# rare-resilience-ai/Osteosarcoma_DiffusionModel

Hardware: AMD Instinct MI355X
Metric: synthetic patients/sec (full T-step reverse sample) (higher is better)
Workload: dtype f32; 1 GPU; reverse sampling of conditional patients, T=1000, D=2000 (50 mut + 1900 expr + 50 pathway), hidden [256,512,256], 3 scenario conditions (BASELINE config 3); patients_per_gpu=100000, T=1000, parallelism=patients sharded over 1 GPU(s), no collective, sampler=chain, chunk_rows=65536, streams=2, graph=True

## Files before the change

### osteosarcoma_diffusionmodel_amd/csrc/gemm_bf3.h

```cpp
#pragma once
#include "gemm_glds.h"
#include "epilogues.h"

namespace osd {

typedef __bf16 bf16x8 __attribute__((ext_vector_type(8)));
typedef __bf16 bf16x2 __attribute__((ext_vector_type(2)));
typedef unsigned v4u32 __attribute__((ext_vector_type(4)));
typedef __attribute__((address_space(1))) v4u32 gv4u32;

constexpr int B3_ROWS = 128;
constexpr int B3_KB = 16;
constexpr int B3_STAGE_U4 = 768;
constexpr int B3_STAGE_BYTES = B3_STAGE_U4 * 16;
constexpr int B3_SLOT_BYTES = 2 * B3_STAGE_BYTES;
#ifndef B3_RING
#define B3_RING 3
#endif
constexpr int B3_SLOTS = B3_RING;
constexpr int B3_LDS_RING_BYTES = B3_SLOTS * B3_SLOT_BYTES;
constexpr int B3_LDS_BYTES = B3_LDS_RING_BYTES + 384 * 4;

inline int64_t b3_tiles(int64_t rows) { return (rows + B3_ROWS - 1) / B3_ROWS; }
inline int b3_nkb(int K) { return (K + B3_KB - 1) / B3_KB; }
inline int64_t b3_units(int64_t rows, int K) { return b3_tiles(rows) * b3_nkb(K) * B3_STAGE_U4; }

struct Bf3Args {
  const uint4* A; int nkb;
  const uint4* B0; int nkb0;
  const uint4* B1; int nkb1;
  int F, P;
  unsigned long long* stamps;
};

__device__ __forceinline__ unsigned pk_bf16(float a, float b) {
  const bf16x2 p = {(__bf16)a, (__bf16)b};
  return __builtin_bit_cast(unsigned, p);
}
__device__ __forceinline__ float bf_lo(unsigned u) { return __uint_as_float(u << 16); }
__device__ __forceinline__ float bf_hi(unsigned u) { return __uint_as_float(u & 0xffff0000u); }

struct Split4 { uint2 p[3]; };
__device__ __forceinline__ Split4 split4(float4 v) {
  Split4 s;
  const unsigned a0 = pk_bf16(v.x, v.y), a1 = pk_bf16(v.z, v.w);
  const float rx = v.x - bf_lo(a0), ry = v.y - bf_hi(a0), rz = v.z - bf_lo(a1), rw = v.w - bf_hi(a1);
  const unsigned b0 = pk_bf16(rx, ry), b1 = pk_bf16(rz, rw);
  const float sx = rx - bf_lo(b0), sy = ry - bf_hi(b0), sz = rz - bf_lo(b1), sw = rw - bf_hi(b1);
  s.p[0] = make_uint2(a0, a1);
  s.p[1] = make_uint2(b0, b1);
  s.p[2] = make_uint2(pk_bf16(sx, sy), pk_bf16(sz, sw));
  return s;
}

__device__ __forceinline__ void stg_u4(uint4* p, uint4 v) { const v4u32 w = {v.x, v.y, v.z, v.w}; *(gv4u32*)p = w; }

__device__ __forceinline__ void b3_put_pair(uint4* __restrict__ o, int kb, int rb, float4 X, float4 Y) {
  const Split4 sx = split4(X), sy = split4(Y);
#pragma unroll
  for (int pl = 0; pl < 3; ++pl) {
    const auto r0 = __builtin_amdgcn_permlane32_swap(sx.p[pl].x, sy.p[pl].x, false, false);
    const auto r1 = __builtin_amdgcn_permlane32_swap(sx.p[pl].y, sy.p[pl].y, false, false);
    stg_u4(o + ((kb * 3 + pl) * 4 + rb) * 64, make_uint4(r0[0], r1[0], r0[1], r1[1]));
  }
}

struct B3Ctx {
  int f0;
  int fl;
  int pt, rb0;
  int p0w;
  int lane, wave;
  int F, P;
  const float* prm;
  float* xreg;
};
constexpr int B3_PRM_FLOATS = 384;

struct B3Out { uint4* planes; int nkb; };

struct B3NoState {};
struct EpiB3Base {
  typedef B3NoState State;
  static constexpr bool LOOP_RNG = false;
  static constexpr bool X_TILE = false;
};

struct EpiB3Bias : EpiB3Base {
  struct Args { const float* bias; float* out; int ldo; };
  static __device__ __forceinline__ const float* prm_ptr(const Args& a, int k) { return k == 0 ? a.bias : nullptr; }
  static __device__ __forceinline__ void apply(f32x16 (&acc)[2][2], const Args& a, const B3Ctx& c, State&) {
    const int l31 = c.lane & 31, h = c.lane >> 5;
#pragma unroll
    for (int fb = 0; fb < 2; ++fb)
#pragma unroll
      for (int q = 0; q < 4; ++q) {
        const int fo = c.fl + 32 * fb + 8 * q + 4 * h;
        const int f = c.f0 + fo;
        const float4 bv = a.bias ? *reinterpret_cast<const float4*>(c.prm + fo) : make_float4(0.f, 0.f, 0.f, 0.f);
        const float b4[4] = {bv.x, bv.y, bv.z, bv.w};
#pragma unroll
        for (int pb = 0; pb < 2; ++pb) {
          const int p = c.p0w + 32 * pb + l31;
          if (p < c.P) {
            float* row = a.out + (size_t)p * a.ldo;
#pragma unroll
            for (int r = 0; r < 4; ++r)
              if (f + r < c.F) row[f + r] = acc[fb][pb][4 * q + r] + b4[r];
          }
        }
      }
  }
};

struct EpiB3Input : EpiB3Base {
  struct Args {
    const float* bias; const float* temb; int ldt; const int* t_index; const int* t_dev; int t_imm;
    const float* cproj; int ldc; B3Out o;
  };
  static __device__ __forceinline__ const float* prm_ptr(const Args& a, int k) {
    if (k == 0) return a.bias;
    if (k == 1 && !a.t_index) return a.temb + (size_t)(a.t_dev ? *a.t_dev : a.t_imm) * a.ldt;
    return nullptr;
  }
  static __device__ __forceinline__ void apply(f32x16 (&acc)[2][2], const Args& a, const B3Ctx& c, State&) {
    const int l31 = c.lane & 31, h = c.lane >> 5;
    uint4* const ob = a.o.planes + (size_t)c.pt * a.o.nkb * B3_STAGE_U4 + c.lane;
#pragma unroll
    for (int pb = 0; pb < 2; ++pb) {
      const int p = c.p0w + 32 * pb + l31;
      const int pc = p < c.P ? p : c.P - 1;
      const float* trow = a.t_index ? a.temb + (size_t)a.t_index[pc] * a.ldt + c.f0 : nullptr;
      const float* crow = a.cproj + (size_t)pc * a.ldc + c.f0;
#pragma unroll
      for (int fb = 0; fb < 2; ++fb)
#pragma unroll
        for (int j = 0; j < 2; ++j) {
          float4 v[2];
#pragma unroll
          for (int e = 0; e < 2; ++e) {
            const int q = 2 * j + e;
            const int fo = c.fl + 32 * fb + 8 * q + 4 * h;
            const float4 bv = *reinterpret_cast<const float4*>(c.prm + fo);
            const float4 tv = trow ? ldg4(trow + fo) : *reinterpret_cast<const float4*>(c.prm + 128 + fo);
            const float4 cv = ldg4(crow + fo);
            v[e].x = ((acc[fb][pb][4 * q] + bv.x) + tv.x) + cv.x;
            v[e].y = ((acc[fb][pb][4 * q + 1] + bv.y) + tv.y) + cv.y;
            v[e].z = ((acc[fb][pb][4 * q + 2] + bv.z) + tv.z) + cv.z;
            v[e].w = ((acc[fb][pb][4 * q + 3] + bv.w) + tv.w) + cv.w;
          }
          b3_put_pair(ob, (c.f0 + c.fl + 32 * fb) / 16 + j, c.rb0 + pb, v[0], v[1]);
        }
    }
  }
};

template <int GW>
struct EpiB3Gn : EpiB3Base {
  struct Args { const float* bias; const float* gamma; const float* beta; B3Out o; };
  static __device__ __forceinline__ const float* prm_ptr(const Args& a, int k) { return k == 0 ? a.bias : (k == 1 ? a.gamma : a.beta); }
  static __device__ __forceinline__ void apply(f32x16 (&acc)[2][2], const Args& a, const B3Ctx& c, B3NoState&) {
    static_assert(GW == 32 || GW == 64, "group widths of the 256 / 512 wide trunk");
    constexpr int RPG = GW / 2;
    constexpr int NG = 32 / RPG;
    const int h = c.lane >> 5;
    uint4* const ob = a.o.planes + (size_t)c.pt * a.o.nkb * B3_STAGE_U4 + c.lane;
#pragma unroll
    for (int fb = 0; fb < 2; ++fb)
#pragma unroll
      for (int q = 0; q < 4; ++q) {
        const float4 bv = *reinterpret_cast<const float4*>(c.prm + c.fl + 32 * fb + 8 * q + 4 * h);
#pragma unroll
        for (int pb = 0; pb < 2; ++pb) {
          acc[fb][pb][4 * q] += bv.x; acc[fb][pb][4 * q + 1] += bv.y;
          acc[fb][pb][4 * q + 2] += bv.z; acc[fb][pb][4 * q + 3] += bv.w;
        }
      }
    float mean[2][NG], rstd[2][NG];
#pragma unroll
    for (int pb = 0; pb < 2; ++pb)
#pragma unroll
      for (int g = 0; g < NG; ++g) {
        float s = 0.f;
#pragma unroll
        for (int j = 0; j < RPG; ++j) { const int Li = g * RPG + j; s += acc[Li / 16][pb][Li % 16]; }
        s += swap_halves(s);
        const float m = s * (1.0f / GW);
        float qs = 0.f;
#pragma unroll
        for (int j = 0; j < RPG; ++j) { const int Li = g * RPG + j; const float d = acc[Li / 16][pb][Li % 16] - m; qs = fmaf(d, d, qs); }
        qs += swap_halves(qs);
        mean[pb][g] = m;
        rstd[pb][g] = 1.0f / sqrtf(qs * (1.0f / GW) + GN_EPS);
      }
#pragma unroll
    for (int fb = 0; fb < 2; ++fb)
#pragma unroll
      for (int j = 0; j < 2; ++j) {
        float4 gv[2], bev[2];
#pragma unroll
        for (int e = 0; e < 2; ++e) {
          const int fo = c.fl + 32 * fb + 8 * (2 * j + e) + 4 * h;
          gv[e] = *reinterpret_cast<const float4*>(c.prm + 128 + fo);
          bev[e] = *reinterpret_cast<const float4*>(c.prm + 256 + fo);
        }
#pragma unroll
        for (int pb = 0; pb < 2; ++pb) {
          float4 y[2];
#pragma unroll
          for (int e = 0; e < 2; ++e) {
            const int q = 2 * j + e;
            const int g = (fb * 16 + 4 * q) / RPG;
            const float m = mean[pb][g], r = rstd[pb][g];
            y[e].x = silu_f(fmaf((acc[fb][pb][4 * q] - m) * r, gv[e].x, bev[e].x));
            y[e].y = silu_f(fmaf((acc[fb][pb][4 * q + 1] - m) * r, gv[e].y, bev[e].y));
            y[e].z = silu_f(fmaf((acc[fb][pb][4 * q + 2] - m) * r, gv[e].z, bev[e].z));
            y[e].w = silu_f(fmaf((acc[fb][pb][4 * q + 3] - m) * r, gv[e].w, bev[e].w));
          }
          b3_put_pair(ob, (c.f0 + c.fl + 32 * fb) / 16 + j, c.rb0 + pb, y[0], y[1]);
        }
      }
  }
};

struct EpiB3Post : EpiB3Base {
  static constexpr bool LOOP_RNG = true;
  static constexpr bool X_TILE = true;
  struct Args {
    const float* bias; float* x; int ldx; const float* coef; const int* t_dev; int t_imm;
    const float* z; int ldzz; long long z_step_stride; int t_first;
    uint64_t seed; uint32_t row_offset; float* mut_mask; int mutation_dim; B3Out o;
    int x_tile;
  };
  struct State { float4 z[16]; int t; };
  static __device__ __forceinline__ const float* prm_ptr(const Args& a, int k) { return k == 0 ? a.bias : nullptr; }
  static __device__ __forceinline__ void init(State& st, const Args& a) { st.t = a.t_dev ? *a.t_dev : a.t_imm; }
  static __device__ __forceinline__ float4 draw(const Args& a, const B3Ctx& c, int t, int i) {
    const int fb = i >> 3, pb = (i >> 2) & 1, q = i & 3;
    const int p = c.p0w + 32 * pb + (c.lane & 31);
    const int f = c.f0 + c.fl + 32 * fb + 8 * q + 4 * (c.lane >> 5);
    return randn4(a.seed, a.row_offset + (uint32_t)p, (uint32_t)(f >> 2), (uint32_t)t, TAG_POSTERIOR);
  }
  static __device__ __forceinline__ bool rng_on(const Args& a, const State& st) { return st.t > 0 && !a.z && a.coef[4 * st.t + 2] != 0.f; }
  static __device__ __forceinline__ void kstep(State& st, const Args& a, const B3Ctx& c, int i) { st.z[i] = draw(a, c, st.t, i); }
  static __device__ __forceinline__ void xtile_issue(const Args& a, const B3Ctx& c) {
    const int rows = c.P - c.p0w;
    const int cmax = (c.F - (c.f0 + c.fl)) / 4 - 1;
    const unsigned dst = __builtin_amdgcn_readfirstlane(lds_addr(c.xreg));
#pragma unroll
    for (int i = 0; i < 16; ++i) {
      const int r = 4 * i + (c.lane >> 4);
      int ch = (c.lane & 15) ^ (r & 15);
      ch = ch < cmax ? ch : (cmax > 0 ? cmax : 0);
      long long row = (long long)c.p0w + (r < rows ? r : rows - 1);
      row = row > 0 ? row : 0;
      int f = c.f0 + c.fl + 4 * ch;
      f = f < c.F - 4 ? f : c.F - 4;
      glds16(a.x + row * a.ldx + f, __builtin_amdgcn_readfirstlane(dst + (unsigned)i * 1024u));
    }
  }
  static __device__ __forceinline__ void apply(f32x16 (&acc)[2][2], const Args& a, const B3Ctx& c, State& st) {
    const int l31 = c.lane & 31, h = c.lane >> 5;
    const int t = st.t;
    const float* cf = a.coef + 4 * t;
    const float cA = cf[0], cB = cf[1], cC = cf[2];
    const float* zbase = a.z ? a.z + (long long)(a.t_first - t) * a.z_step_stride : nullptr;
    const bool do_mask = t == 0 && a.mut_mask != nullptr;
    const bool zal = zbase && (a.ldzz & 3) == 0 && (reinterpret_cast<uintptr_t>(zbase) & 15) == 0;
    const int f0w = c.f0 + c.fl;
    uint4* const ob = a.o.planes + (size_t)c.pt * a.o.nkb * B3_STAGE_U4 + c.lane;
#pragma unroll
    for (int fb = 0; fb < 2; ++fb)
#pragma unroll
      for (int q = 0; q < 4; ++q) {
        const int fo = c.fl + 32 * fb + 8 * q + 4 * h;
        const int f = c.f0 + fo;
        const float4 b4 = *reinterpret_cast<const float4*>(c.prm + fo);
        const float bv[4] = {b4.x, b4.y, b4.z, b4.w};
#pragma unroll
        for (int pb = 0; pb < 2; ++pb) {
          float zv[4] = {0.f, 0.f, 0.f, 0.f};
          if (t > 0 && cC != 0.f) {
            if (zbase) {
              const int p = c.p0w + 32 * pb + l31;
              const size_t zo = (size_t)(p < c.P ? p : c.P - 1) * a.ldzz;
              if (zal && f + 3 < c.F) { const float4 z4 = ldg4(zbase + zo + f); zv[0] = z4.x; zv[1] = z4.y; zv[2] = z4.z; zv[3] = z4.w; }
              else {
#pragma unroll
                for (int r = 0; r < 4; ++r) zv[r] = f + r < c.F ? zbase[zo + f + r] : 0.f;
              }
            } else {
              const float4 z4 = st.z[(fb * 2 + pb) * 4 + q];
              zv[0] = z4.x; zv[1] = z4.y; zv[2] = z4.z; zv[3] = z4.w;
            }
          }
#pragma unroll
          for (int r = 0; r < 4; ++r) acc[fb][pb][4 * q + r] = fmaf(cB, acc[fb][pb][4 * q + r] + bv[r], cC * zv[r]);
        }
      }
    if (a.x_tile) asm volatile("s_waitcnt vmcnt(0)" ::: "memory");
#pragma unroll
    for (int fb = 0; fb < 2; ++fb) {
      if (f0w + 32 * fb >= c.F) break;
#pragma unroll
      for (int pb = 0; pb < 2; ++pb) {
        const int rl = 32 * pb + l31;
        const int p = c.p0w + rl;
        const bool prow = p < c.P;
        const int pc = prow ? p : c.P - 1;
        float* xrow = a.x + (size_t)pc * a.ldx;
#pragma unroll
        for (int j = 0; j < 2; ++j) {
          if (f0w + 32 * fb + 16 * j >= c.F) break;
          float4 o[2];
#pragma unroll
          for (int e = 0; e < 2; ++e) {
            const int q = 2 * j + e;
            const int fo = c.fl + 32 * fb + 8 * q + 4 * h;
            const int f = c.f0 + fo;
            float xv[4];
            float* xs = nullptr;
            if (a.x_tile) {
              xs = c.xreg + rl * 64 + 4 * ((8 * fb + 2 * q + h) ^ (rl & 15));
              const float4 x4 = *reinterpret_cast<const float4*>(xs);
              xv[0] = x4.x; xv[1] = x4.y; xv[2] = x4.z; xv[3] = x4.w;
            } else {
#pragma unroll
              for (int r = 0; r < 4; ++r) xv[r] = f + r < c.F ? xrow[f + r] : 0.f;
            }
            float ov[4];
#pragma unroll
            for (int r = 0; r < 4; ++r) {
              ov[r] = fmaf(cA, xv[r], acc[fb][pb][4 * q + r]);
              if (f + r >= c.F) ov[r] = 0.f;
            }
            if (do_mask && prow && f < a.mutation_dim) {
              float* mrow = a.mut_mask + (size_t)p * a.mutation_dim;
#pragma unroll
              for (int r = 0; r < 4; ++r)
                if (f + r < a.mutation_dim) mrow[f + r] = (ov[r] > 0.5f) ? 1.0f : 0.0f;
            }
            o[e] = make_float4(ov[0], ov[1], ov[2], ov[3]);
            if (a.x_tile) *reinterpret_cast<float4*>(xs) = o[e];
            else if (prow) {
#pragma unroll
              for (int r = 0; r < 4; ++r)
                if (f + r < c.F) xrow[f + r] = ov[r];
            }
          }
          b3_put_pair(ob, (f0w + 32 * fb) / 16 + j, c.rb0 + pb, o[0], o[1]);
        }
      }
    }
    if (a.x_tile) {
      const int rows = c.P - c.p0w;
      const int nch = (c.F - f0w) / 4;
#pragma unroll
      for (int i0 = 0; i0 < 16; i0 += 4) {
        float4 v[4];
#pragma unroll
        for (int k = 0; k < 4; ++k) v[k] = *reinterpret_cast<const float4*>(c.xreg + (i0 + k) * 256 + c.lane * 4);
#pragma unroll
        for (int k = 0; k < 4; ++k) {
          const int r = 4 * (i0 + k) + (c.lane >> 4);
          const int ch = (c.lane & 15) ^ (r & 15);
          if (r < rows && ch < nch) stg4(a.x + (size_t)(c.p0w + r) * a.ldx + f0w + 4 * ch, v[k]);
        }
      }
    }
  }
};

struct B3Frags { uint4 a[2][3], b[2][3]; };
#ifndef B3_LD
#define B3_LD 0
#endif
#ifndef B3_SGB_VALU
#define B3_SGB_VALU 5
#endif
#ifndef B3_EXP
#define B3_EXP 0
#endif

template <int N>
__device__ __forceinline__ void glds16s_run(gfloat_ptr sbase, unsigned voff, unsigned lds_dst) {
  static_assert(N == 3 || N == 4, "runs of 3 or 4 pieces (instruction offsets up to 3072)");
  unsigned keep;
  if constexpr (N == 3)
    asm volatile(
        "s_mov_b32 %0, m0\n\ts_mov_b32 m0, %3\n\ts_nop 4\n\t"
        "global_load_lds_dwordx4 %1, %2\n\tglobal_load_lds_dwordx4 %1, %2 offset:1024\n\tglobal_load_lds_dwordx4 %1, %2 offset:2048\n\t"
        "s_mov_b32 m0, %0"
        : "=&s"(keep) : "v"(voff), "s"(sbase), "s"(lds_dst) : "memory");
  else
    asm volatile(
        "s_mov_b32 %0, m0\n\ts_mov_b32 m0, %3\n\ts_nop 4\n\t"
        "global_load_lds_dwordx4 %1, %2\n\tglobal_load_lds_dwordx4 %1, %2 offset:1024\n\tglobal_load_lds_dwordx4 %1, %2 offset:2048\n\t"
        "global_load_lds_dwordx4 %1, %2 offset:3072\n\t"
        "s_mov_b32 m0, %0"
        : "=&s"(keep) : "v"(voff), "s"(sbase), "s"(lds_dst) : "memory");
}
__device__ __forceinline__ void glds4(const float* gsrc, unsigned lds_dst) {
  unsigned keep;
  asm volatile(
      "s_mov_b32 %0, m0\n\ts_mov_b32 m0, %2\n\ts_nop 0\n\tglobal_load_lds_dword %1, off\n\ts_mov_b32 m0, %0"
      : "=&s"(keep) : "v"(gsrc), "s"(lds_dst) : "memory");
}
template <int N> __device__ __forceinline__ void b3_wait_vm() {
  static_assert(N == 0 || N == 6 || N == 12 || N == 24, "");
  if constexpr (N == 0) asm volatile("s_waitcnt vmcnt(0)" ::: "memory");
  else if constexpr (N == 6) asm volatile("s_waitcnt vmcnt(6)" ::: "memory");
  else if constexpr (N == 12) asm volatile("s_waitcnt vmcnt(12)" ::: "memory");
  else asm volatile("s_waitcnt vmcnt(24)" ::: "memory");
}

template <class Epi, int LD, int NKB = 0>
__global__ __launch_bounds__(NTHREADS + 64 * LD, (LD || B3_RING == 2) ? 3 : 2) void gemm_bf3_kernel(Bf3Args g, typename Epi::Args ea) {
  static_assert(LD == 0 || LD == 2, "no loader waves, or one per operand");
  static_assert(NKB == 0 || NKB == 16 || NKB == 32, "unrolled lengths: 256 / 512 deep reductions");
  extern __shared__ __attribute__((aligned(16))) uint4 b3smem[];
  const int nft = (g.F + B3_ROWS - 1) / B3_ROWS;
  const int npt = (g.P + B3_ROWS - 1) / B3_ROWS;
  const int b = blockIdx.x;
  const int idx = b >> 3;
  const int ft = idx % nft;
  const int pt = (idx / nft) * 8 + (b & 7);
  if (pt >= npt) return;
  const int pt_src = (B3_EXP & 2) ? 0 : pt;

  const int tid = threadIdx.x;
  const int lane = tid & 63;
  const int wave = __builtin_amdgcn_readfirstlane(tid >> 6);
  const bool loader = LD > 0 && wave >= 4;
  const int rbA = ((wave >> 1) & 1) * 2;
  const int rbB = (wave & 1) * 2;

  const int nkb = NKB ? NKB : g.nkb;
  const gfloat_ptr Ag = uniform_ptr(reinterpret_cast<const float*>(g.A + (size_t)ft * nkb * B3_STAGE_U4));
  const gfloat_ptr B0g = uniform_ptr(reinterpret_cast<const float*>(g.B0 + (size_t)pt_src * g.nkb0 * B3_STAGE_U4));
  const gfloat_ptr B1g = uniform_ptr(reinterpret_cast<const float*>(g.B1 ? g.B1 + (size_t)pt_src * g.nkb1 * B3_STAGE_U4 : g.B0));
  const int nkb0 = g.nkb0;
  const unsigned voff = (unsigned)lane * 16u;
  const unsigned lds0 = __builtin_amdgcn_readfirstlane(lds_addr(reinterpret_cast<const float*>(b3smem)));
  float* const prm = reinterpret_cast<float*>(b3smem) + B3_LDS_RING_BYTES / 4;
  unsigned long long st_c = 0, st_r = 0;
  if (g.stamps) { st_c = __builtin_amdgcn_s_memtime(); st_r = __builtin_amdgcn_s_memrealtime(); }

  if (wave < 3) {
    const float* src = Epi::prm_ptr(ea, wave);
    if (src) {
      const int f0 = ft * B3_ROWS;
#pragma unroll
      for (int i = 0; i < 2; ++i) {
        int f = f0 + 64 * i + lane;
        f = f < g.F ? f : g.F - 1;
        glds4(src + f, __builtin_amdgcn_readfirstlane(lds_addr(prm) + (unsigned)wave * 512u + (unsigned)i * 256u));
      }
    }
  }

  auto issue_stage = [&](int st, int sl) {
    const gfloat_ptr as = Ag + (size_t)st * (B3_STAGE_BYTES / 4);
    const gfloat_ptr bs = st < nkb0 ? B0g + (size_t)st * (B3_STAGE_BYTES / 4) : B1g + (size_t)(st - nkb0) * (B3_STAGE_BYTES / 4);
    const unsigned dst = lds0 + (unsigned)sl * (unsigned)B3_SLOT_BYTES;
    if constexpr (LD == 0) {
      glds16s_run<3>(as + wave * 768, voff, __builtin_amdgcn_readfirstlane(dst + (unsigned)wave * 3072u));
      glds16s_run<3>(bs + wave * 768, voff, __builtin_amdgcn_readfirstlane(dst + (unsigned)B3_STAGE_BYTES + (unsigned)wave * 3072u));
    } else {
      const gfloat_ptr src = wave == 4 ? as : bs;
      const unsigned d = __builtin_amdgcn_readfirstlane(dst + (wave == 4 ? 0u : (unsigned)B3_STAGE_BYTES));
#pragma unroll
      for (int i = 0; i < 3; ++i) glds16s_run<4>(src + i * 1024, voff, __builtin_amdgcn_readfirstlane(d + (unsigned)i * 4096u));
    }
  };
  constexpr int PPS = LD ? 12 : 6;
  auto read_frags = [&](B3Frags& f, int sl) {
    const uint4* s = b3smem + sl * (B3_SLOT_BYTES / 16) + lane;
#pragma unroll
    for (int pl = 0; pl < 3; ++pl)
#pragma unroll
      for (int i = 0; i < 2; ++i) {
        f.a[i][pl] = s[(pl * 4 + rbA + i) * 64];
        f.b[i][pl] = s[B3_STAGE_U4 + (pl * 4 + rbB + i) * 64];
      }
  };

  int s0 = 0, s1 = 1, s2 = 2;
  if (loader) {
    issue_stage(0, 0);
    if (nkb > 1) issue_stage(1, 1);
    if (nkb > 2) issue_stage(2, 2);
    if (nkb > 2) b3_wait_vm<2 * PPS>(); else if (nkb > 1) b3_wait_vm<PPS>(); else b3_wait_vm<0>();
    asm volatile("s_barrier" ::: "memory");
    if (nkb > 2) b3_wait_vm<PPS>(); else b3_wait_vm<0>();
    asm volatile("s_barrier" ::: "memory");
    for (int s = 0; s < nkb; ++s) {
      const bool more = s + 3 < nkb && !(B3_EXP & 1);
      if (more) { issue_stage(s + 3, s0); b3_wait_vm<PPS>(); } else b3_wait_vm<0>();
      if (!(B3_EXP & 8)) asm volatile("s_barrier" ::: "memory");
      const int k = s0; s0 = s1; s1 = s2; s2 = k;
    }
    return;
  }

  f32x16 acc[2][2];
#pragma unroll
  for (int i = 0; i < 2; ++i)
#pragma unroll
    for (int j = 0; j < 2; ++j)
#pragma unroll
      for (int r = 0; r < 16; ++r) acc[i][j][r] = 0.f;

  B3Ctx ctx;
  ctx.f0 = ft * B3_ROWS; ctx.fl = rbA * 32; ctx.pt = pt; ctx.rb0 = rbB; ctx.p0w = pt * B3_ROWS + rbB * 32;
  ctx.lane = lane; ctx.wave = wave; ctx.F = g.F; ctx.P = g.P; ctx.prm = prm;
  ctx.xreg = reinterpret_cast<float*>(b3smem) + wave * 4096;
  typename Epi::State est;
  bool rng = false;
  if constexpr (Epi::LOOP_RNG) { Epi::init(est, ea); rng = NKB > 0 && Epi::rng_on(ea, est); }
  bool xt = false;
  if constexpr (Epi::X_TILE) xt = ea.x_tile != 0 && B3_RING == 3;

  auto mfma_block = [&](const B3Frags& f, bool draw, int rs) {
    constexpr int PA[6] = {2, 1, 0, 1, 0, 0};
    constexpr int PB[6] = {0, 1, 2, 0, 1, 0};
#pragma unroll
    for (int t = 0; t < 6; ++t)
#pragma unroll
      for (int i = 0; i < 2; ++i)
#pragma unroll
        for (int j = 0; j < 2; ++j)
          acc[i][j] = __builtin_amdgcn_mfma_f32_32x32x16_bf16(__builtin_bit_cast(bf16x8, f.a[i][PA[t]]), __builtin_bit_cast(bf16x8, f.b[j][PB[t]]),
                                                              acc[i][j], 0, 0, 0);
    if constexpr (NKB > 0 && Epi::LOOP_RNG) {
      if (draw) {
        Epi::kstep(est, ea, ctx, rs);
#ifndef B3_NO_SGB
#pragma unroll
        for (int k = 0; k < 24; ++k) {
          __builtin_amdgcn_sched_group_barrier(0x008, 1, 0);
          __builtin_amdgcn_sched_group_barrier(0x002, B3_SGB_VALU, 0);
        }
#endif
      }
    }
  };

  B3Frags f0, f1;
  if constexpr (LD == 0) {
    issue_stage(0, 0);
    if (nkb > 1) issue_stage(1, 1);
    if (nkb > 2 && B3_RING == 3) issue_stage(2, 2);
    if (nkb > 2 && B3_RING == 3) b3_wait_vm<2 * PPS>(); else if (nkb > 1) b3_wait_vm<PPS>(); else b3_wait_vm<0>();
  }
  asm volatile("s_barrier" ::: "memory");
  read_frags(f0, 0);
  if constexpr (LD == 0) { if (nkb > 2 && B3_RING == 3) b3_wait_vm<PPS>(); else b3_wait_vm<0>(); }
  __builtin_amdgcn_s_waitcnt(0xC07F);
  asm volatile("s_barrier" ::: "memory");

  auto step = [&](const B3Frags& cur, B3Frags& nxt, int s) {
    __builtin_amdgcn_sched_barrier(0);
    const bool last = s + 1 >= nkb;
    const bool more = LD == 0 && s + B3_RING < nkb && !(B3_EXP & 1);
    if (more) issue_stage(s + B3_RING, s0);
    if constexpr (Epi::X_TILE) {
      if (last && xt) Epi::xtile_issue(ea, ctx);
    }
    __builtin_amdgcn_sched_barrier(0);
    if (!last && !(B3_EXP & 4)) read_frags(nxt, s1);
    __builtin_amdgcn_sched_barrier(0);
    mfma_block((B3_EXP & 4) ? f0 : cur, rng && (NKB == 16 || !(s & 1)), NKB == 16 ? s : s / 2);
    __builtin_amdgcn_sched_barrier(0);
    if constexpr (LD == 0) {
      if (more && B3_RING == 3) b3_wait_vm<PPS>();
      else if (!(Epi::X_TILE && last && xt)) b3_wait_vm<0>();
    }
    __builtin_amdgcn_s_waitcnt(0xC07F);
    if (!(B3_EXP & 8)) asm volatile("s_barrier" ::: "memory");
    if (B3_RING == 3) { const int k = s0; s0 = s1; s1 = s2; s2 = k; }
    else { const int k = s0; s0 = s1; s1 = k; }
  };
  if constexpr (NKB > 0) {
#pragma unroll
    for (int s = 0; s < NKB; s += 2) {
      step(f0, f1, s);
      step(f1, f0, s + 1);
    }
  } else {
    for (int s = 0; s < nkb; s += 2) {
      step(f0, f1, s);
      if (s + 1 < nkb) step(f1, f0, s + 1);
    }
  }
  unsigned long long st_k = 0;
  if (g.stamps) {
    st_k = __builtin_amdgcn_s_memtime();
    if (tid == 0) {
      unsigned long long* o = g.stamps + (size_t)blockIdx.x * 4;
      o[0] = st_k - st_c;
      o[1] = __builtin_amdgcn_s_memrealtime() - st_r;
    }
  }
  if constexpr (Epi::LOOP_RNG) {
    if (!rng && Epi::rng_on(ea, est)) {
#pragma unroll
      for (int i = 0; i < 16; ++i) Epi::kstep(est, ea, ctx, i);
    }
  }
  Epi::apply(acc, ea, ctx, est);
  if (g.stamps) {
    asm volatile("s_waitcnt vmcnt(0)" ::: "memory");
    if (tid == 0) g.stamps[(size_t)blockIdx.x * 4 + 2] = __builtin_amdgcn_s_memtime() - st_k;
  }
}

}
```

Measured before the change: 22940 patients/s.

## Use nontemporal plane/x stores, scalar-base x loads, and an RNG-specialized K loop

Plane and x writebacks in the fused posterior epilogue now use nontemporal stores. The x-tile prefetch now uses a scalar base pointer plus a per-lane offset, issued as an nt global_load_lds. The K loop is duplicated into compile-time draw and no-draw versions, which removes the runtime rng check from every step. Noise draws are reordered and pinned with an asm barrier, and the VALU count per sched group drops from 5 to 3. The aim is less cache pollution, lower address-computation cost and a tighter MFMA/VALU interleave, at the cost of larger code and possible changes to cache reuse for data read soon after.

```diff
diff --git a/osteosarcoma_diffusionmodel_amd/csrc/gemm_bf3.h b/osteosarcoma_diffusionmodel_amd/csrc/gemm_bf3.h
--- a/osteosarcoma_diffusionmodel_amd/csrc/gemm_bf3.h
+++ b/osteosarcoma_diffusionmodel_amd/csrc/gemm_bf3.h
@@ -54,14 +54,23 @@
 }
 
 __device__ __forceinline__ void stg_u4(uint4* p, uint4 v) { const v4u32 w = {v.x, v.y, v.z, v.w}; *(gv4u32*)p = w; }
-
+__device__ __forceinline__ void stg_u4_nt(uint4* p, uint4 v) { const v4u32 w = {v.x, v.y, v.z, v.w}; __builtin_nontemporal_store(w, (gv4u32*)p); }
+__device__ __forceinline__ void stg4_nt(float* p, float4 v) { const v4f32 w = {v.x, v.y, v.z, v.w}; __builtin_nontemporal_store(w, (gfloat4*)p); }
+__device__ __forceinline__ void glds16s_nt(gfloat_ptr sbase, unsigned voff, unsigned lds_dst) {
+  unsigned keep;
+  asm volatile("s_mov_b32 %0, m0\n\ts_mov_b32 m0, %3\n\ts_nop 4\n\tglobal_load_lds_dwordx4 %1, %2 nt\n\ts_mov_b32 m0, %0"
+               : "=&s"(keep) : "v"(voff), "s"(sbase), "s"(lds_dst) : "memory");
+}
+
+template <bool NT = false>
 __device__ __forceinline__ void b3_put_pair(uint4* __restrict__ o, int kb, int rb, float4 X, float4 Y) {
   const Split4 sx = split4(X), sy = split4(Y);
 #pragma unroll
   for (int pl = 0; pl < 3; ++pl) {
     const auto r0 = __builtin_amdgcn_permlane32_swap(sx.p[pl].x, sy.p[pl].x, false, false);
     const auto r1 = __builtin_amdgcn_permlane32_swap(sx.p[pl].y, sy.p[pl].y, false, false);
-    stg_u4(o + ((kb * 3 + pl) * 4 + rb) * 64, make_uint4(r0[0], r1[0], r0[1], r1[1]));
+    if constexpr (NT) stg_u4_nt(o + ((kb * 3 + pl) * 4 + rb) * 64, make_uint4(r0[0], r1[0], r0[1], r1[1]));
+    else stg_u4(o + ((kb * 3 + pl) * 4 + rb) * 64, make_uint4(r0[0], r1[0], r0[1], r1[1]));
   }
 }
 
@@ -242,21 +251,28 @@
     return randn4(a.seed, a.row_offset + (uint32_t)p, (uint32_t)(f >> 2), (uint32_t)t, TAG_POSTERIOR);
   }
   static __device__ __forceinline__ bool rng_on(const Args& a, const State& st) { return st.t > 0 && !a.z && a.coef[4 * st.t + 2] != 0.f; }
-  static __device__ __forceinline__ void kstep(State& st, const Args& a, const B3Ctx& c, int i) { st.z[i] = draw(a, c, st.t, i); }
+  static __device__ __forceinline__ void kstep(State& st, const Args& a, const B3Ctx& c, int k) {
+    const int i = ((((k >> 2) & 1) * 2 + (k >> 3)) * 4) + (k & 3);
+    float4 z = draw(a, c, st.t, i);
+    asm volatile("" : "+v"(z.x), "+v"(z.y), "+v"(z.z), "+v"(z.w));
+    st.z[i] = z;
+  }
   static __device__ __forceinline__ void xtile_issue(const Args& a, const B3Ctx& c) {
     const int rows = c.P - c.p0w;
     const int cmax = (c.F - (c.f0 + c.fl)) / 4 - 1;
     const unsigned dst = __builtin_amdgcn_readfirstlane(lds_addr(c.xreg));
+    const int rbase = c.p0w < c.P ? c.p0w : c.P - 1;
+    const gfloat_ptr xb = uniform_ptr(a.x + (size_t)rbase * a.ldx);
+    const int rlast = rows > 0 ? rows - 1 : 0;
 #pragma unroll
     for (int i = 0; i < 16; ++i) {
       const int r = 4 * i + (c.lane >> 4);
       int ch = (c.lane & 15) ^ (r & 15);
       ch = ch < cmax ? ch : (cmax > 0 ? cmax : 0);
-      long long row = (long long)c.p0w + (r < rows ? r : rows - 1);
-      row = row > 0 ? row : 0;
+      const int rr = r < rlast ? r : rlast;
       int f = c.f0 + c.fl + 4 * ch;
       f = f < c.F - 4 ? f : c.F - 4;
-      glds16(a.x + row * a.ldx + f, __builtin_amdgcn_readfirstlane(dst + (unsigned)i * 1024u));
+      glds16s_nt(xb, (unsigned)(rr * a.ldx + f) * 4u, __builtin_amdgcn_readfirstlane(dst + (unsigned)i * 1024u));
     }
   }
   static __device__ __forceinline__ void apply(f32x16 (&acc)[2][2], const Args& a, const B3Ctx& c, State& st) {
@@ -348,7 +364,7 @@
                 if (f + r < c.F) xrow[f + r] = ov[r];
             }
           }
-          b3_put_pair(ob, (f0w + 32 * fb) / 16 + j, c.rb0 + pb, o[0], o[1]);
+          b3_put_pair<true>(ob, (f0w + 32 * fb) / 16 + j, c.rb0 + pb, o[0], o[1]);
         }
       }
     }
@@ -364,7 +380,7 @@
         for (int k = 0; k < 4; ++k) {
           const int r = 4 * (i0 + k) + (c.lane >> 4);
           const int ch = (c.lane & 15) ^ (r & 15);
-          if (r < rows && ch < nch) stg4(a.x + (size_t)(c.p0w + r) * a.ldx + f0w + 4 * ch, v[k]);
+          if (r < rows && ch < nch) stg4_nt(a.x + (size_t)(c.p0w + r) * a.ldx + f0w + 4 * ch, v[k]);
         }
       }
     }
@@ -372,11 +388,12 @@
 };
 
 struct B3Frags { uint4 a[2][3], b[2][3]; };
+template <bool V> struct B3Const { static constexpr bool value = V; };
 #ifndef B3_LD
 #define B3_LD 0
 #endif
 #ifndef B3_SGB_VALU
-#define B3_SGB_VALU 5
+#define B3_SGB_VALU 3
 #endif
 #ifndef B3_EXP
 #define B3_EXP 0
@@ -521,7 +538,7 @@
   bool xt = false;
   if constexpr (Epi::X_TILE) xt = ea.x_tile != 0 && B3_RING == 3;
 
-  auto mfma_block = [&](const B3Frags& f, bool draw, int rs) {
+  auto mfma_block = [&](const B3Frags& f, bool draw, int rs) __attribute__((always_inline)) {
     constexpr int PA[6] = {2, 1, 0, 1, 0, 0};
     constexpr int PB[6] = {0, 1, 2, 0, 1, 0};
 #pragma unroll
@@ -559,7 +576,8 @@
   __builtin_amdgcn_s_waitcnt(0xC07F);
   asm volatile("s_barrier" ::: "memory");
 
-  auto step = [&](const B3Frags& cur, B3Frags& nxt, int s) {
+  auto step = [&](const B3Frags& cur, B3Frags& nxt, int s, auto draw_c) __attribute__((always_inline)) {
+    constexpr bool DRAW = decltype(draw_c)::value;
     __builtin_amdgcn_sched_barrier(0);
     const bool last = s + 1 >= nkb;
     const bool more = LD == 0 && s + B3_RING < nkb && !(B3_EXP & 1);
@@ -570,7 +588,7 @@
     __builtin_amdgcn_sched_barrier(0);
     if (!last && !(B3_EXP & 4)) read_frags(nxt, s1);
     __builtin_amdgcn_sched_barrier(0);
-    mfma_block((B3_EXP & 4) ? f0 : cur, rng && (NKB == 16 || !(s & 1)), NKB == 16 ? s : s / 2);
+    mfma_block((B3_EXP & 4) ? f0 : cur, DRAW && (NKB == 16 || !(s & 1)), NKB == 16 ? s : s / 2);
     __builtin_amdgcn_sched_barrier(0);
     if constexpr (LD == 0) {
       if (more && B3_RING == 3) b3_wait_vm<PPS>();
@@ -582,15 +600,20 @@
     else { const int k = s0; s0 = s1; s1 = k; }
   };
   if constexpr (NKB > 0) {
-#pragma unroll
-    for (int s = 0; s < NKB; s += 2) {
-      step(f0, f1, s);
-      step(f1, f0, s + 1);
-    }
+    auto kloop = [&](auto draw_c) __attribute__((always_inline)) {
+#pragma unroll
+      for (int s = 0; s < NKB; s += 2) {
+        step(f0, f1, s, draw_c);
+        step(f1, f0, s + 1, draw_c);
+      }
+    };
+    if constexpr (Epi::LOOP_RNG) {
+      if (rng) kloop(B3Const<true>{}); else kloop(B3Const<false>{});
+    } else kloop(B3Const<false>{});
   } else {
     for (int s = 0; s < nkb; s += 2) {
-      step(f0, f1, s);
-      if (s + 1 < nkb) step(f1, f0, s + 1);
+      step(f0, f1, s, B3Const<false>{});
+      if (s + 1 < nkb) step(f1, f0, s + 1, B3Const<false>{});
     }
   }
   unsigned long long st_k = 0;
@@ -602,8 +625,8 @@
       o[1] = __builtin_amdgcn_s_memrealtime() - st_r;
     }
   }
-  if constexpr (Epi::LOOP_RNG) {
-    if (!rng && Epi::rng_on(ea, est)) {
+  if constexpr (Epi::LOOP_RNG && NKB == 0) {
+    if (Epi::rng_on(ea, est)) {
 #pragma unroll
       for (int i = 0; i < 16; ++i) Epi::kstep(est, ea, ctx, i);
     }
```

After: 22950 patients/s (median of 2 runs). Within noise of the previous version (+0.1%).
